# ORNL/DDStore

Hardware: AMD Instinct MI355X
Metric: samples/sec (global-shuffle sample fetch) (higher is better)
Workload: dtype bf16; 1 GPU; model=store-globalshuffle-fetch, global_batch=262144, rows_per_rank=2097152, row_bytes=512, store_dtype=f32, parallelism=dp1, mode=fetch

## Files before the change

### ddstore_amd/csrc/ddstore.hpp

```cpp
#pragma once

#include <torch/extension.h>

#include <hip/hip_runtime.h>
#include <c10/hip/HIPStream.h>
#include <ATen/Parallel.h>

#include <fcntl.h>
#include <sys/mman.h>
#include <unistd.h>

#if defined(__x86_64__)
#include <emmintrin.h>
#endif

#include <atomic>
#include <condition_variable>
#include <cstdlib>
#include <cstring>
#include <exception>
#include <functional>
#include <map>
#include <mutex>
#include <string>
// ... 417 lines not shown
                TORCH_CHECK(e == hipSuccess,
                            "ddstore open_peers: hipIpcOpenMemHandle failed for peer rank ",
                            r, " (", hipGetErrorString(e),
                            ") -- peers must share one node/xGMI domain and "
                            "HSA_ENABLE_IPC_MODE_LEGACY=0 must be set");
                v.peers[r] = p;
                v.opened[r] = 1;
            }
        }
        size_t nb = nparts_ * sizeof(void*) + (nparts_ + 1) * 8 +
                    (v.is_csr ? (nparts_ + 1) * 8 : 0) + DDS_NCTR * 8;
        HIP_CHECK(hipMalloc((void**)&v.d_peers, nb));
        v.d_prefix = reinterpret_cast<int64_t*>(v.d_peers + nparts_);
        HIP_CHECK(hipMemcpy(v.d_peers, v.peers.data(), nparts_ * sizeof(void*),
                            hipMemcpyHostToDevice));
        HIP_CHECK(hipMemcpy(v.d_prefix, v.prefix.data(), (nparts_ + 1) * 8,
                            hipMemcpyHostToDevice));
        int64_t* tail = v.d_prefix + nparts_ + 1;
        if (v.is_csr) {
            v.d_elem_prefix = tail;
            HIP_CHECK(hipMemcpy(v.d_elem_prefix, v.elem_prefix.data(),
                                (nparts_ + 1) * 8, hipMemcpyHostToDevice));
            tail += nparts_ + 1;
        }
        v.d_oob = reinterpret_cast<unsigned long long*>(tail);
        HIP_CHECK(hipMemset(v.d_oob, 0, DDS_NCTR * 8));
    }

    void update(const std::string& name, const at::Tensor& src, int64_t offset) {
        DeviceVar& v = var(name);
        TORCH_CHECK(!v.is_csr, "ddstore update: not supported for CSR variables");
        TORCH_CHECK(src.is_contiguous(), "ddstore update: array must be C-contiguous");
        TORCH_CHECK(dds_itemsize(dds_type_of(src)) == v.itemsize,
                    "ddstore update: itemsize mismatch");
        int64_t nrows = src.numel() / v.row_elems;
        TORCH_CHECK(src.numel() == nrows * v.row_elems, "ddstore update: shape mismatch");
        TORCH_CHECK(offset >= 0 && offset + nrows <= v.nrows_local,
                    "ddstore update: out of range");
        ingest(v.base, src, offset * v.row_elems * v.itemsize);
    }

    void get_range(const std::string& name, int64_t start, int64_t count,
                   at::Tensor out) {
        DeviceVar& v = var(name);
        TORCH_CHECK(!v.is_csr, "ddstore get: use get_csr for CSR variables");
        TORCH_CHECK(out.is_contiguous(), "ddstore get: output must be C-contiguous");
        TORCH_CHECK(dds_itemsize(dds_type_of(out)) == v.itemsize,
                    "ddstore get: itemsize mismatch");
        TORCH_CHECK(out.numel() == count * v.row_elems, "ddstore get: shape mismatch");
        check_peers(v);
        int64_t ntotal = v.prefix[nparts_];
        TORCH_CHECK(start >= 0 && start < ntotal, "Invalid start on target");
        int target = owner_of_host(v.prefix, start);
        TORCH_CHECK(start + count <= v.prefix[target + 1], "Invalid count on target");
        const char* src = (const char*)v.peers[target] +
                          (start - v.prefix[target]) * v.row_elems * v.itemsize;
        size_t nb = (size_t)count * v.row_elems * v.itemsize;
        if (out.device().is_cpu()) {
            HIP_CHECK(hipStreamSynchronize(stream()));
            HIP_CHECK(hipMemcpy(out.data_ptr(), src, nb, hipMemcpyDeviceToHost));
        } else {
            TORCH_CHECK(out.device().index() == device_, "ddstore get: wrong device");
            HIP_CHECK(hipMemcpyAsync(out.data_ptr(), src, nb,
                                     hipMemcpyDeviceToDevice, stream()));
        }
        v.n_gather += 1;
        v.rows_gathered += count;
        v.bytes_gathered += nb;
    }

    void gather(const std::string& name, const at::Tensor& idx, at::Tensor out) {
        RoctxRange rr_("ddstore::gather");
        DeviceVar& v = var(name);
        TORCH_CHECK(!v.is_csr, "ddstore gather: use gather_csr for CSR variables");
        check_peers(v);
        check_idx(idx);
        int64_t nidx = idx.numel();
        TORCH_CHECK(out.is_contiguous() && out.device().is_cuda() &&
                        out.device().index() == device_,
                    "ddstore gather: output must be a contiguous tensor on the store device");
        TORCH_CHECK(out.numel() == nidx * v.row_elems, "ddstore gather: shape mismatch");
        int out_t = dds_type_of(out);
        ddstore::gather_rows(stream(), (const void* const*)v.d_peers, v.d_prefix,
                             nparts_, idx.data_ptr<int64_t>(), nidx, v.row_elems,
                             v.dds_t, out_t, out.data_ptr(), v.d_oob);
        v.n_gather += 1;
        v.rows_gathered += nidx;
        v.bytes_gathered += nidx * v.row_elems * v.itemsize;
    }

    void gather_affine(const std::string& name, const at::Tensor& idx,
                       at::Tensor out, double scale, double shift) {
        RoctxRange rr_("ddstore::gather_affine");
        DeviceVar& v = var(name);
        TORCH_CHECK(!v.is_csr, "ddstore gather: use gather_csr for CSR variables");
        check_peers(v);
        check_idx(idx);
        int64_t nidx = idx.numel();
        TORCH_CHECK(out.is_contiguous() && out.device().is_cuda() &&
                        out.device().index() == device_,
                    "ddstore gather: output must be a contiguous tensor on the store device");
        TORCH_CHECK(out.numel() == nidx * v.row_elems, "ddstore gather: shape mismatch");
        int out_t = dds_type_of(out);
        TORCH_CHECK(out_t == DDS_F32 || out_t == DDS_F16 || out_t == DDS_BF16,
                    "ddstore gather: affine output must be f32/f16/bf16");
        ddstore::gather_rows_affine(stream(), (const void* const*)v.d_peers,
                                    v.d_prefix, nparts_, idx.data_ptr<int64_t>(),
                                    nidx, v.row_elems, v.dds_t, out_t,
                                    (float)scale, (float)shift, out.data_ptr(),
                                    v.d_oob);
        v.n_gather += 1;
        v.rows_gathered += nidx;
        v.bytes_gathered += nidx * v.row_elems * v.itemsize;
    }

    void gather_csr(const std::string& name, const at::Tensor& idx,
                    const at::Tensor& out_off, at::Tensor out, int64_t total_elems) {
        RoctxRange rr_("ddstore::gather_csr");
        DeviceVar& v = var(name);
        TORCH_CHECK(v.is_csr, "ddstore gather_csr: not a CSR variable");
        check_peers(v);
        check_idx(idx);
        check_idx(out_off);
        int64_t nidx = idx.numel();
        TORCH_CHECK(out_off.numel() == nidx + 1, "ddstore gather_csr: bad out_off");
        TORCH_CHECK(out.is_contiguous() && out.device().is_cuda() &&
                        dds_type_of(out) == v.dds_t,
                    "ddstore gather_csr: bad output tensor");
        TORCH_CHECK(out.numel() >= total_elems * v.row_elems,
                    "ddstore gather_csr: output too small");
        const int64_t cap = out.numel() / std::max<int64_t>(v.row_elems, 1);
        ddstore::gather_csr(stream(), (const void* const*)v.d_peers, v.d_prefix,
                            v.d_elem_prefix, nparts_, v.d_goff,
                            idx.data_ptr<int64_t>(), nidx,
                            out_off.data_ptr<int64_t>(),
                            v.row_elems * v.itemsize, cap,
                            out.data_ptr(), v.d_oob);
        v.n_gather += 1;
        v.rows_gathered += nidx;
        v.bytes_gathered += total_elems * v.row_elems * v.itemsize;
    }

    at::Tensor gather_csr_fast(const std::string& name, const at::Tensor& idx,
                               at::Tensor out) {
        RoctxRange rr_("ddstore::gather_csr_fast");
        DeviceVar& v = var(name);
        TORCH_CHECK(v.is_csr, "ddstore gather_csr: not a CSR variable");
        check_peers(v);
        check_idx(idx);
        const int64_t nidx = idx.numel();
        TORCH_CHECK(out.is_contiguous() && out.device().is_cuda() &&
                        dds_type_of(out) == v.dds_t,
                    "ddstore gather_csr: bad output tensor");
        auto opts = at::TensorOptions().dtype(at::kLong).device(idx.device());
        at::Tensor off = at::empty({nidx + 1}, opts);
        if (nidx == 0) {
            off.zero_();
            return off;
        }
        const int64_t cap = out.numel() / std::max<int64_t>(v.row_elems, 1);
        const int64_t elem_bytes = v.row_elems * v.itemsize;
        auto bopts = at::TensorOptions().dtype(at::kByte).device(idx.device());
        at::Tensor scratch = at::empty(
            {(int64_t)ddstore::csr_plan_scratch_bytes(nidx)}, bopts);
        const int64_t desc_cap =
            cap / ddstore::csr_item_elems(elem_bytes) + nidx;
        at::Tensor desc = at::empty({2 * desc_cap}, opts);
        ddstore::gather_csr_balanced(
            stream(), (const void* const*)v.d_peers, v.d_prefix,
            v.d_elem_prefix, nparts_, v.d_goff, v.prefix[nparts_],
            idx.data_ptr<int64_t>(), nidx, elem_bytes, cap,
            off.data_ptr<int64_t>(), out.data_ptr(), v.d_oob,
            scratch.data_ptr(), desc.data_ptr<int64_t>(), desc_cap);
        v.n_gather += 1;
        v.rows_gathered += nidx;
        return off;
    }

    void csr_lens(const std::string& name, const at::Tensor& idx, at::Tensor lens) {
        DeviceVar& v = var(name);
        TORCH_CHECK(v.is_csr, "ddstore csr_lens: not a CSR variable");
        check_peers(v);
        check_idx(idx);
        TORCH_CHECK(lens.scalar_type() == at::kLong && lens.is_contiguous() &&
                        lens.device().is_cuda() && lens.numel() == idx.numel(),
                    "ddstore csr_lens: bad lens tensor");
        ddstore::csr_lens(stream(), v.d_goff, idx.data_ptr<int64_t>(), idx.numel(),
                          v.prefix[nparts_], lens.data_ptr<int64_t>(), v.d_oob,
                          nullptr);
    }
// ... 686 lines not shown
```

### ddstore_amd/csrc/ddstore_kernels.h

```cpp
#pragma once

#include <hip/hip_runtime.h>
#include <cstdint>

enum DDSType : int {
    DDS_U8 = 0,
    DDS_I32 = 1,
    DDS_I64 = 2,
    DDS_F32 = 3,
    DDS_F64 = 4,
    DDS_F16 = 5,
    DDS_BF16 = 6,
    DDS_F8E4M3 = 7,
    DDS_F8E5M2 = 8,
    DDS_NUM_TYPES = 9
};

#define DDS_MAX_PARTS 128

#define DDS_CTR_OOB 0
#define DDS_CTR_CAP 1
#define DDS_CTR_ELEMS 2
#define DDS_NCTR 3

namespace ddstore {

void gather_rows(hipStream_t stream,
                 const void* const* d_peer_base,
                 const int64_t* d_prefix, int nparts,
                 const int64_t* d_idx, int64_t nidx,
                 int64_t row_elems, int in_t, int out_t,
                 void* d_out, unsigned long long* d_oob);

void gather_rows_affine(hipStream_t stream,
                        const void* const* d_peer_base,
                        const int64_t* d_prefix, int nparts,
                        const int64_t* d_idx, int64_t nidx,
                        int64_t row_elems, int in_t, int out_t,
                        float scale, float shift,
                        void* d_out, unsigned long long* d_oob);

void gather_csr(hipStream_t stream,
                const void* const* d_peer_base,
                const int64_t* d_sample_prefix,
                const int64_t* d_elem_prefix, int nparts,
                const int64_t* d_goff,
                const int64_t* d_idx, int64_t nidx,
                const int64_t* d_out_off,
                int64_t elem_bytes, int64_t cap_elems,
                void* d_out, unsigned long long* d_ctrs);

void csr_lens(hipStream_t stream, const int64_t* d_goff, const int64_t* d_idx,
              int64_t nidx, int64_t nsamples, int64_t* d_lens,
              unsigned long long* d_oob, unsigned long long* d_elems);

size_t csr_plan_scratch_bytes(int64_t nidx);
int64_t csr_item_elems(int64_t elem_bytes);
void gather_csr_balanced(hipStream_t stream, const void* const* d_peer_base,
                         const int64_t* d_sample_prefix,
                         const int64_t* d_elem_prefix, int nparts,
                         const int64_t* d_goff, int64_t nsamples_total,
                         const int64_t* d_idx, int64_t nidx,
                         int64_t elem_bytes, int64_t cap_elems,
                         int64_t* d_out_off, void* d_out,
                         unsigned long long* d_ctrs,
                         void* d_scratch, int64_t* d_desc, int64_t desc_cap);


void scatter_rows_local(hipStream_t stream,
                        void* d_base, int64_t nrows_local,
                        int64_t row_elems, int elem_t,
                        const int64_t* d_local_idx, int64_t nidx,
                        const void* d_src, unsigned long long* d_oob);

}
```

### ddstore_amd/csrc/ddstore_kernels.hip

```cpp

#include "ddstore_kernels.h"

#include <hip/hip_fp16.h>
#include <hip/hip_bf16.h>
#include <hip/hip_fp8.h>
#include <type_traits>
#include <cstdlib>

namespace ddstore {

namespace {

constexpr int kBlock = 256;
constexpr int64_t kMaxBlocks = 32768;

inline int n_blocks(int64_t work_items) {
    int64_t b = (work_items + kBlock - 1) / kBlock;
    if (b < 1) b = 1;
    if (b > kMaxBlocks) b = kMaxBlocks;
    return (int)b;
}

template <typename T, int N>
struct alignas(sizeof(T) * N) VecT {
    T v[N];
};

__device__ __forceinline__ int owner_of(const int64_t* prefix, int nparts, int64_t row) {
    int lo = 0, hi = nparts - 1;
    while (lo < hi) {
        int mid = (lo + hi + 1) >> 1;
        if (prefix[mid] <= row) lo = mid; else hi = mid - 1;
    }
    return lo;
}

template <typename T>
constexpr bool is_fp8_v =
    std::is_same_v<T, __hip_fp8_e4m3> || std::is_same_v<T, __hip_fp8_e5m2>;

template <typename Tout, typename Tin>
__device__ __forceinline__ Tout cvt(Tin v) {
    if constexpr (std::is_same_v<Tout, Tin>) {
        return v;
    } else if constexpr (std::is_same_v<Tin, __half>) {
        return cvt<Tout, float>(__half2float(v));
    } else if constexpr (std::is_same_v<Tin, __hip_bfloat16>) {
        return cvt<Tout, float>(__bfloat162float(v));
    } else if constexpr (is_fp8_v<Tin>) {
        return cvt<Tout, float>(static_cast<float>(v));
    } else if constexpr (std::is_same_v<Tout, __half>) {
        return __float2half(static_cast<float>(v));
    } else if constexpr (std::is_same_v<Tout, __hip_bfloat16>) {
        return __float2bfloat16(static_cast<float>(v));
    } else if constexpr (is_fp8_v<Tout>) {
        return Tout(static_cast<float>(v));
    } else {
        return static_cast<Tout>(v);
    }
}

template <int CHUNK>
__global__ void __launch_bounds__(kBlock)
k_gather_rows_b16(const void* const* peer_base, const int64_t* gprefix, int nparts,
                  const int64_t* idx, int64_t nidx, int64_t chunks_per_row,
                  uint4* __restrict__ out, unsigned long long* oob) {
    using V = VecT<uint4, CHUNK / 16>;
    __shared__ int64_t s_prefix[DDS_MAX_PARTS + 1];
    __shared__ const V* s_base[DDS_MAX_PARTS];
    for (int i = threadIdx.x; i <= nparts; i += kBlock) s_prefix[i] = gprefix[i];
    for (int i = threadIdx.x; i < nparts; i += kBlock)
        s_base[i] = reinterpret_cast<const V*>(peer_base[i]);
    __syncthreads();

    V* __restrict__ vout = reinterpret_cast<V*>(out);
    const int64_t total = nidx * chunks_per_row;
    for (int64_t t = (int64_t)blockIdx.x * kBlock + threadIdx.x; t < total;
         t += (int64_t)gridDim.x * kBlock) {
        const int64_t r = t / chunks_per_row;
        const int64_t c = t - r * chunks_per_row;
        const int64_t g = idx[r];
        if (g < 0 || g >= s_prefix[nparts]) {
            if (c == 0) atomicAdd(oob, 1ull);
            continue;
        }
        const int p = owner_of(s_prefix, nparts, g);
        vout[t] = s_base[p][(g - s_prefix[p]) * chunks_per_row + c];
    }
}

template <typename Tin, typename Tout>
__global__ void __launch_bounds__(kBlock)
k_gather_rows_castv(const void* const* peer_base, const int64_t* gprefix, int nparts,
                    const int64_t* idx, int64_t nidx, int64_t row_elems,
                    Tout* __restrict__ out, unsigned long long* oob) {
    constexpr int VEC = 16 / sizeof(Tout);
    using Vin = VecT<Tin, VEC>;
    using Vout = VecT<Tout, VEC>;
    __shared__ int64_t s_prefix[DDS_MAX_PARTS + 1];
    __shared__ const Tin* s_base[DDS_MAX_PARTS];
    for (int i = threadIdx.x; i <= nparts; i += kBlock) s_prefix[i] = gprefix[i];
    for (int i = threadIdx.x; i < nparts; i += kBlock)
        s_base[i] = reinterpret_cast<const Tin*>(peer_base[i]);
    __syncthreads();

    const int64_t cpr = row_elems / VEC;
    const int64_t total = nidx * cpr;
    for (int64_t t = (int64_t)blockIdx.x * kBlock + threadIdx.x; t < total;
         t += (int64_t)gridDim.x * kBlock) {
        const int64_t r = t / cpr;
        const int64_t c = t - r * cpr;
        const int64_t g = idx[r];
        if (g < 0 || g >= s_prefix[nparts]) {
            if (c == 0) atomicAdd(oob, 1ull);
            continue;
        }
        const int p = owner_of(s_prefix, nparts, g);
        const Vin vin = *reinterpret_cast<const Vin*>(
            s_base[p] + (g - s_prefix[p]) * row_elems + c * VEC);
        Vout vout;
#pragma unroll
        for (int k = 0; k < VEC; ++k) vout.v[k] = cvt<Tout>(vin.v[k]);
        *reinterpret_cast<Vout*>(out + t * VEC) = vout;
    }
}

template <typename T>
__device__ __forceinline__ float to_f32(T v) {
    if constexpr (std::is_same_v<T, __half>) return __half2float(v);
    else if constexpr (std::is_same_v<T, __hip_bfloat16>) return __bfloat162float(v);
    else if constexpr (is_fp8_v<T>) return static_cast<float>(v);
    else return (float)v;
}

template <typename Tin, typename Tout>
__global__ void __launch_bounds__(kBlock)
k_gather_rows_affine(const void* const* peer_base, const int64_t* gprefix, int nparts,
                     const int64_t* idx, int64_t nidx, int64_t row_elems,
                     float scale, float shift,
                     Tout* __restrict__ out, unsigned long long* oob) {
    constexpr int VEC = 16 / sizeof(Tout);
    using Vin = VecT<Tin, VEC>;
    using Vout = VecT<Tout, VEC>;
    __shared__ int64_t s_prefix[DDS_MAX_PARTS + 1];
    __shared__ const Tin* s_base[DDS_MAX_PARTS];
    for (int i = threadIdx.x; i <= nparts; i += kBlock) s_prefix[i] = gprefix[i];
    for (int i = threadIdx.x; i < nparts; i += kBlock)
        s_base[i] = reinterpret_cast<const Tin*>(peer_base[i]);
    __syncthreads();

    const int64_t cpr = row_elems / VEC;
    const int64_t total = nidx * cpr;
    for (int64_t t = (int64_t)blockIdx.x * kBlock + threadIdx.x; t < total;
         t += (int64_t)gridDim.x * kBlock) {
        const int64_t r = t / cpr;
        const int64_t c = t - r * cpr;
        const int64_t g = idx[r];
        if (g < 0 || g >= s_prefix[nparts]) {
            if (c == 0) atomicAdd(oob, 1ull);
            continue;
        }
        const int p = owner_of(s_prefix, nparts, g);
        const Vin vin = *reinterpret_cast<const Vin*>(
            s_base[p] + (g - s_prefix[p]) * row_elems + c * VEC);
        Vout vout;
#pragma unroll
        for (int k = 0; k < VEC; ++k)
            vout.v[k] = cvt<Tout>(fmaf(to_f32(vin.v[k]), scale, shift));
        *reinterpret_cast<Vout*>(out + t * VEC) = vout;
    }
}

template <typename Tin, typename Tout>
__global__ void __launch_bounds__(kBlock)
k_gather_rows_affine_s(const void* const* peer_base, const int64_t* gprefix, int nparts,
                       const int64_t* idx, int64_t nidx, int64_t row_elems,
                       float scale, float shift,
                       Tout* __restrict__ out, unsigned long long* oob) {
    __shared__ int64_t s_prefix[DDS_MAX_PARTS + 1];
    __shared__ const Tin* s_base[DDS_MAX_PARTS];
    for (int i = threadIdx.x; i <= nparts; i += kBlock) s_prefix[i] = gprefix[i];
    for (int i = threadIdx.x; i < nparts; i += kBlock)
        s_base[i] = reinterpret_cast<const Tin*>(peer_base[i]);
    __syncthreads();
    const int64_t total = nidx * row_elems;
    for (int64_t t = (int64_t)blockIdx.x * kBlock + threadIdx.x; t < total;
         t += (int64_t)gridDim.x * kBlock) {
        const int64_t r = t / row_elems;
        const int64_t c = t - r * row_elems;
        const int64_t g = idx[r];
        if (g < 0 || g >= s_prefix[nparts]) {
            if (c == 0) atomicAdd(oob, 1ull);
            continue;
        }
        const int p = owner_of(s_prefix, nparts, g);
        out[t] = cvt<Tout>(fmaf(
            to_f32(s_base[p][(g - s_prefix[p]) * row_elems + c]), scale, shift));
    }
}

template <typename Tin, typename Tout>
__global__ void __launch_bounds__(kBlock)
k_gather_rows_cast(const void* const* peer_base, const int64_t* gprefix, int nparts,
                   const int64_t* idx, int64_t nidx, int64_t row_elems,
                   Tout* __restrict__ out, unsigned long long* oob) {
    __shared__ int64_t s_prefix[DDS_MAX_PARTS + 1];
    __shared__ const Tin* s_base[DDS_MAX_PARTS];
    for (int i = threadIdx.x; i <= nparts; i += kBlock) s_prefix[i] = gprefix[i];
    for (int i = threadIdx.x; i < nparts; i += kBlock)
        s_base[i] = reinterpret_cast<const Tin*>(peer_base[i]);
    __syncthreads();

    const int64_t total = nidx * row_elems;
    for (int64_t t = (int64_t)blockIdx.x * kBlock + threadIdx.x; t < total;
         t += (int64_t)gridDim.x * kBlock) {
        const int64_t r = t / row_elems;
        const int64_t c = t - r * row_elems;
        const int64_t g = idx[r];
        if (g < 0 || g >= s_prefix[nparts]) {
            if (c == 0) atomicAdd(oob, 1ull);
            continue;
        }
        const int p = owner_of(s_prefix, nparts, g);
        out[t] = cvt<Tout>(s_base[p][(g - s_prefix[p]) * row_elems + c]);
    }
}

template <typename T, int GROUP>
__global__ void __launch_bounds__(kBlock)
k_gather_csr_wave(const void* const* peer_base,
                  const int64_t* sample_prefix, const int64_t* elem_prefix, int nparts,
                  const int64_t* goff,
                  const int64_t* idx, int64_t nidx,
                  const int64_t* out_off, int64_t chunks_per_elem,
                  int64_t cap_elems,
                  T* __restrict__ out, unsigned long long* ctrs) {
    __shared__ int64_t s_sprefix[DDS_MAX_PARTS + 1];
    __shared__ int64_t s_eprefix[DDS_MAX_PARTS + 1];
    __shared__ const T* s_base[DDS_MAX_PARTS];
    for (int i = threadIdx.x; i <= nparts; i += kBlock) {
        s_sprefix[i] = sample_prefix[i];
        s_eprefix[i] = elem_prefix[i];
    }
    for (int i = threadIdx.x; i < nparts; i += kBlock)
        s_base[i] = reinterpret_cast<const T*>(peer_base[i]);
    __syncthreads();

    constexpr int GPB = kBlock / GROUP;
    const int64_t first = (int64_t)blockIdx.x * GPB + threadIdx.x / GROUP;
    const int64_t step = (int64_t)gridDim.x * GPB;
    const int tid = threadIdx.x % GROUP;
    for (int64_t s = first; s < nidx; s += step) {
// ... 315 lines not shown
                   const int64_t* __restrict__ desc,
                   const int64_t* __restrict__ meta,
                   void* __restrict__ out_, unsigned long long* ctrs) {
    __shared__ const char* s_base[DDS_MAX_PARTS];
    for (int i = threadIdx.x; i < nparts; i += kBlock)
        s_base[i] = reinterpret_cast<const char*>(peer_base[i]);
    __syncthreads();
    const int64_t total = meta[0];
    constexpr int GPB = kBlock / GROUP;
    const int64_t first = (int64_t)blockIdx.x * GPB + threadIdx.x / GROUP;
    const int64_t step = (int64_t)gridDim.x * GPB;
    const int tid = threadIdx.x % GROUP;
    (void)ctrs;
    for (int64_t j = first; j < total; j += step) {
        const int64_t d0 = desc[2 * j];
        const int64_t d1 = desc[2 * j + 1];
        const int p = (int)(d0 >> 56);
        const int64_t src_u = d0 & ((int64_t(1) << 56) - 1);
        const int64_t n_u = d1 >> 44;
        const int64_t dst_u = d1 & ((int64_t(1) << 44) - 1);
        if constexpr (DW) {
            copy_dwords_store16<VAR>(
                reinterpret_cast<uint32_t*>(out_) + dst_u,
                reinterpret_cast<const uint32_t*>(s_base[p]) + src_u,
                n_u, tid, GROUP);
        } else {
            char* dst = reinterpret_cast<char*>(out_) + dst_u;
            const char* src = s_base[p] + src_u;
            for (int64_t c = tid; c < n_u; c += GROUP) dst[c] = src[c];
        }
    }
}

template <int CHUNK>
__global__ void __launch_bounds__(kBlock)
k_scatter_rows_b16(uint4* __restrict__ base_, int64_t nrows, int64_t chunks_per_row,
                   const int64_t* local_idx, int64_t nidx,
                   const uint4* __restrict__ src_, unsigned long long* oob) {
    using V = VecT<uint4, CHUNK / 16>;
    V* __restrict__ base = reinterpret_cast<V*>(base_);
    const V* __restrict__ src = reinterpret_cast<const V*>(src_);
    const int64_t total = nidx * chunks_per_row;
    for (int64_t t = (int64_t)blockIdx.x * kBlock + threadIdx.x; t < total;
         t += (int64_t)gridDim.x * kBlock) {
        const int64_t r = t / chunks_per_row;
        const int64_t c = t - r * chunks_per_row;
        const int64_t l = local_idx[r];
        if (l < 0 || l >= nrows) {
            if (c == 0) atomicAdd(oob, 1ull);
            continue;
        }
        base[l * chunks_per_row + c] = src[t];
    }
}

template <typename T>
__global__ void __launch_bounds__(kBlock)
k_scatter_rows_elem(T* __restrict__ base, int64_t nrows, int64_t row_elems,
                    const int64_t* local_idx, int64_t nidx,
                    const T* __restrict__ src, unsigned long long* oob) {
    const int64_t total = nidx * row_elems;
    for (int64_t t = (int64_t)blockIdx.x * kBlock + threadIdx.x; t < total;
         t += (int64_t)gridDim.x * kBlock) {
        const int64_t r = t / row_elems;
        const int64_t c = t - r * row_elems;
        const int64_t l = local_idx[r];
        if (l < 0 || l >= nrows) {
            if (c == 0) atomicAdd(oob, 1ull);
            continue;
        }
        base[l * row_elems + c] = src[t];
    }
}

inline int dds_itemsize(int t) {
    switch (t) {
        case DDS_U8: case DDS_F8E4M3: case DDS_F8E5M2: return 1;
        case DDS_F16: case DDS_BF16: return 2;
        case DDS_I32: case DDS_F32: return 4;
        default: return 8;
    }
}

template <typename Tin, typename Tout>
void launch_gather_cast_one(hipStream_t stream, const void* const* pb,
                            const int64_t* pf, int np, const int64_t* idx,
                            int64_t n, int64_t re, Tout* out,
                            unsigned long long* oob) {
    constexpr int VEC = 16 / sizeof(Tout);
    if (re % VEC == 0 && ((uintptr_t)out % 16) == 0) {
        const int grid = n_blocks(n * (re / VEC));
        hipLaunchKernelGGL((k_gather_rows_castv<Tin, Tout>), dim3(grid), dim3(kBlock),
                           0, stream, pb, pf, np, idx, n, re, out, oob);
    } else {
        const int grid = n_blocks(n * re);
        hipLaunchKernelGGL((k_gather_rows_cast<Tin, Tout>), dim3(grid), dim3(kBlock),
                           0, stream, pb, pf, np, idx, n, re, out, oob);
    }
}

template <typename Tin>
void launch_gather_cast_out(hipStream_t stream, const void* const* pb,
                            const int64_t* pf, int np, const int64_t* idx,
                            int64_t n, int64_t re, int out_t, void* out,
                            unsigned long long* oob) {
    switch (out_t) {
#define DDS_OUT(tag, T)                                                               \
    case tag:                                                                         \
        launch_gather_cast_one<Tin, T>(stream, pb, pf, np, idx, n, re, (T*)out, oob); \
        break;
        DDS_OUT(DDS_U8, uint8_t)
        DDS_OUT(DDS_I32, int32_t)
        DDS_OUT(DDS_I64, int64_t)
        DDS_OUT(DDS_F32, float)
        DDS_OUT(DDS_F64, double)
        DDS_OUT(DDS_F16, __half)
        DDS_OUT(DDS_BF16, __hip_bfloat16)
        DDS_OUT(DDS_F8E4M3, __hip_fp8_e4m3)
        DDS_OUT(DDS_F8E5M2, __hip_fp8_e5m2)
#undef DDS_OUT
    }
}

}

template <typename Tin>
void launch_affine_out(hipStream_t stream, const void* const* pb, const int64_t* pf,
                       int np, const int64_t* idx, int64_t n, int64_t re,
                       float a, float b, int out_t, void* out,
                       unsigned long long* oob) {
#define DDS_AFF(tag, T)                                                              \
    case tag: {                                                                      \
        constexpr int VEC = 16 / sizeof(T);                                          \
        if (re % VEC == 0 && ((uintptr_t)out % 16) == 0) {                           \
            const int grid = n_blocks(n * (re / VEC));                               \
            hipLaunchKernelGGL((k_gather_rows_affine<Tin, T>), dim3(grid),           \
                               dim3(kBlock), 0, stream, pb, pf, np, idx, n, re, a,   \
                               b, (T*)out, oob);                                     \
        } else {                                                                     \
            const int grid = n_blocks(n * re);                                       \
            hipLaunchKernelGGL((k_gather_rows_affine_s<Tin, T>), dim3(grid),         \
                               dim3(kBlock), 0, stream, pb, pf, np, idx, n, re, a,   \
                               b, (T*)out, oob);                                     \
        }                                                                            \
        break;                                                                       \
    }
    switch (out_t) {
        DDS_AFF(DDS_F32, float)
        DDS_AFF(DDS_F16, __half)
        DDS_AFF(DDS_BF16, __hip_bfloat16)
    }
#undef DDS_AFF
}

void gather_rows_affine(hipStream_t stream,
                        const void* const* d_peer_base,
                        const int64_t* d_prefix, int nparts,
                        const int64_t* d_idx, int64_t nidx,
                        int64_t row_elems, int in_t, int out_t,
                        float scale, float shift,
                        void* d_out, unsigned long long* d_oob) {
    if (nidx == 0 || row_elems == 0) return;
    switch (in_t) {
#define DDS_AIN(tag, T)                                                          \
    case tag:                                                                    \
        launch_affine_out<T>(stream, d_peer_base, d_prefix, nparts, d_idx,       \
                             nidx, row_elems, scale, shift, out_t, d_out,        \
                             d_oob);                                             \
        break;
        DDS_AIN(DDS_U8, uint8_t)
        DDS_AIN(DDS_I32, int32_t)
        DDS_AIN(DDS_I64, int64_t)
        DDS_AIN(DDS_F32, float)
        DDS_AIN(DDS_F64, double)
        DDS_AIN(DDS_F16, __half)
        DDS_AIN(DDS_BF16, __hip_bfloat16)
        DDS_AIN(DDS_F8E4M3, __hip_fp8_e4m3)
        DDS_AIN(DDS_F8E5M2, __hip_fp8_e5m2)
#undef DDS_AIN
    }
}

void gather_rows(hipStream_t stream,
                 const void* const* d_peer_base,
                 const int64_t* d_prefix, int nparts,
                 const int64_t* d_idx, int64_t nidx,
                 int64_t row_elems, int in_t, int out_t,
                 void* d_out, unsigned long long* d_oob) {
    if (nidx == 0 || row_elems == 0) return;
    const int64_t row_bytes = row_elems * dds_itemsize(in_t);
    const uintptr_t out_align = (uintptr_t)d_out;
    if (in_t == out_t && row_bytes % 16 == 0 && out_align % 16 == 0) {
        const int64_t cpr = row_bytes / 16;
        if (row_bytes % 32 == 0 && row_bytes >= 128 && out_align % 32 == 0) {
            const int64_t cpr32 = row_bytes / 32;
            const int grid = n_blocks(nidx * cpr32);
            hipLaunchKernelGGL((k_gather_rows_b16<32>), dim3(grid), dim3(kBlock), 0,
                               stream, d_peer_base, d_prefix, nparts, d_idx, nidx,
                               cpr32, (uint4*)d_out, d_oob);
        } else {
            const int grid = n_blocks(nidx * cpr);
            hipLaunchKernelGGL((k_gather_rows_b16<16>), dim3(grid), dim3(kBlock), 0,
                               stream, d_peer_base, d_prefix, nparts, d_idx, nidx,
                               cpr, (uint4*)d_out, d_oob);
        }
        return;
    }
    switch (in_t) {
#define DDS_IN(tag, T)                                                           \
    case tag:                                                                    \
        launch_gather_cast_out<T>(stream, d_peer_base, d_prefix, nparts, d_idx,  \
                                  nidx, row_elems, out_t, d_out, d_oob);         \
        break;
        DDS_IN(DDS_U8, uint8_t)
        DDS_IN(DDS_I32, int32_t)
        DDS_IN(DDS_I64, int64_t)
        DDS_IN(DDS_F32, float)
        DDS_IN(DDS_F64, double)
        DDS_IN(DDS_F16, __half)
        DDS_IN(DDS_BF16, __hip_bfloat16)
        DDS_IN(DDS_F8E4M3, __hip_fp8_e4m3)
        DDS_IN(DDS_F8E5M2, __hip_fp8_e5m2)
#undef DDS_IN
    }
}

void csr_lens(hipStream_t stream, const int64_t* d_goff, const int64_t* d_idx,
              int64_t nidx, int64_t nsamples, int64_t* d_lens,
              unsigned long long* d_oob, unsigned long long* d_elems) {
    if (nidx == 0) return;
    hipLaunchKernelGGL(k_csr_lens, dim3(n_blocks(nidx)), dim3(kBlock), 0, stream,
                       d_goff, d_idx, nidx, nsamples, d_lens, d_oob, d_elems);
}


void gather_csr(hipStream_t stream,
                const void* const* d_peer_base,
                const int64_t* d_sample_prefix,
                const int64_t* d_elem_prefix, int nparts,
                const int64_t* d_goff,
                const int64_t* d_idx, int64_t nidx,
                const int64_t* d_out_off,
                int64_t elem_bytes, int64_t cap_elems,
                void* d_out, unsigned long long* d_ctrs) {
    if (nidx == 0) return;
    static const int g_override = [] {
        const char* e = getenv("DDSTORE_CSR_GROUP");
        return e ? atoi(e) : 0;
    }();
    int group = nidx >= 16384 ? 16 : (nidx >= 4096 ? 64 : 256);
    if (g_override) group = g_override;
    int64_t b = (nidx + (kBlock / group) - 1) / (kBlock / group);
    const int grid = (int)(b < kMaxBlocks ? b : kMaxBlocks);
    const uintptr_t oa = (uintptr_t)d_out;
#define DDS_CSR_G(T, div, G)                                                         \
    hipLaunchKernelGGL((k_gather_csr_wave<T, G>), dim3(grid), dim3(kBlock), 0,       \
                       stream, d_peer_base, d_sample_prefix, d_elem_prefix, nparts,  \
                       d_goff, d_idx, nidx, d_out_off, elem_bytes / div, cap_elems,  \
                       (T*)d_out, d_ctrs)
#define DDS_CSR_T(T, div)                                                            \
    do {                                                                             \
        if (group == 8) DDS_CSR_G(T, div, 8);                                        \
        else if (group == 16) DDS_CSR_G(T, div, 16);                                  \
        else if (group == 32) DDS_CSR_G(T, div, 32);                                 \
        else if (group == 64) DDS_CSR_G(T, div, 64);                                 \
        else DDS_CSR_G(T, div, 256);                                                 \
    } while (0)
    static const int copy_var = [] {
        const char* e = getenv("DDSTORE_CSR_COPY");
        int v = e ? atoi(e) : 0;
        return (v >= 0 && v <= 2) ? v : 0;
    }();
#define DDS_CSR_DW_V(G, V)                                                           \
    hipLaunchKernelGGL((k_gather_csr_dw<G, V>), dim3(grid), dim3(kBlock), 0, stream, \
                       d_peer_base, d_sample_prefix, d_elem_prefix, nparts, d_goff,  \
                       d_idx, nidx, d_out_off, elem_bytes / 4, cap_elems,            \
                       (uint32_t*)d_out, d_ctrs)
#define DDS_CSR_DW(G)                                                                \
    do {                                                                             \
        if (copy_var == 0) DDS_CSR_DW_V(G, 0);                                       \
        else if (copy_var == 2) DDS_CSR_DW_V(G, 2);                                  \
        else DDS_CSR_DW_V(G, 1);                                                     \
    } while (0)
    if (elem_bytes % 16 == 0 && oa % 16 == 0) {
        DDS_CSR_T(uint4, 16);
    } else if (elem_bytes % 4 == 0 && oa % 4 == 0) {
        if (group == 8) DDS_CSR_DW(8);
        else if (group == 16) DDS_CSR_DW(16);
        else if (group == 32) DDS_CSR_DW(32);
        else if (group == 64) DDS_CSR_DW(64);
        else DDS_CSR_DW(256);
    } else {
        DDS_CSR_T(uint8_t, 1);
    }
// ... 117 lines not shown
```

Before: 6.240 billion samples/s.

## Add wave-tiled gather kernel with kernel-arg directory and nontemporal stores

Adds a new gather kernel in which each wavefront handles a tile of rows. It loads the row indices once per lane, prefetches the next tile's indices, resolves each row's owner partition from a directory passed as kernel arguments (for up to 8 parts) instead of a shared-memory binary search, and broadcasts source pointers with shuffles. Loads are unrolled and outputs use nontemporal 16-byte stores. The identity, cast and affine gather paths all route to this kernel by default, with environment knobs to fall back. The aim is to cut per-element index loads, directory lookups and the cost of the integer division in the old grid-stride kernel. In exchange the grid is limited to 8 blocks per CU, which may reduce memory parallelism.

```diff
diff --git a/ddstore_amd/csrc/ddstore.hpp b/ddstore_amd/csrc/ddstore.hpp
--- a/ddstore_amd/csrc/ddstore.hpp
+++ b/ddstore_amd/csrc/ddstore.hpp
@@ -523,6 +523,7 @@
         TORCH_CHECK(out.numel() == nidx * v.row_elems, "ddstore gather: shape mismatch");
         int out_t = dds_type_of(out);
         ddstore::gather_rows(stream(), (const void* const*)v.d_peers, v.d_prefix,
+                             (const void* const*)v.peers.data(), v.prefix.data(),
                              nparts_, idx.data_ptr<int64_t>(), nidx, v.row_elems,
                              v.dds_t, out_t, out.data_ptr(), v.d_oob);
         v.n_gather += 1;
@@ -546,7 +547,8 @@
         TORCH_CHECK(out_t == DDS_F32 || out_t == DDS_F16 || out_t == DDS_BF16,
                     "ddstore gather: affine output must be f32/f16/bf16");
         ddstore::gather_rows_affine(stream(), (const void* const*)v.d_peers,
-                                    v.d_prefix, nparts_, idx.data_ptr<int64_t>(),
+                                    v.d_prefix, (const void* const*)v.peers.data(),
+                                    v.prefix.data(), nparts_, idx.data_ptr<int64_t>(),
                                     nidx, v.row_elems, v.dds_t, out_t,
                                     (float)scale, (float)shift, out.data_ptr(),
                                     v.d_oob);
diff --git a/ddstore_amd/csrc/ddstore_kernels.h b/ddstore_amd/csrc/ddstore_kernels.h
--- a/ddstore_amd/csrc/ddstore_kernels.h
+++ b/ddstore_amd/csrc/ddstore_kernels.h
@@ -23,18 +23,29 @@
 #define DDS_CTR_ELEMS 2
 #define DDS_NCTR 3
 
+#define DDS_DIR_KPARTS 8
+
 namespace ddstore {
+
+struct GatherDirK {
+    int64_t prefix[DDS_DIR_KPARTS + 1];
+    const void* base[DDS_DIR_KPARTS];
+};
 
 void gather_rows(hipStream_t stream,
                  const void* const* d_peer_base,
-                 const int64_t* d_prefix, int nparts,
+                 const int64_t* d_prefix,
+                 const void* const* h_peer_base,
+                 const int64_t* h_prefix, int nparts,
                  const int64_t* d_idx, int64_t nidx,
                  int64_t row_elems, int in_t, int out_t,
                  void* d_out, unsigned long long* d_oob);
 
 void gather_rows_affine(hipStream_t stream,
                         const void* const* d_peer_base,
-                        const int64_t* d_prefix, int nparts,
+                        const int64_t* d_prefix,
+                        const void* const* h_peer_base,
+                        const int64_t* h_prefix, int nparts,
                         const int64_t* d_idx, int64_t nidx,
                         int64_t row_elems, int in_t, int out_t,
                         float scale, float shift,
diff --git a/ddstore_amd/csrc/ddstore_kernels.hip b/ddstore_amd/csrc/ddstore_kernels.hip
--- a/ddstore_amd/csrc/ddstore_kernels.hip
+++ b/ddstore_amd/csrc/ddstore_kernels.hip
@@ -6,6 +6,7 @@
 #include <hip/hip_fp8.h>
 #include <type_traits>
 #include <cstdlib>
+#include <string>
 
 namespace ddstore {
 
@@ -168,6 +169,182 @@
         for (int k = 0; k < VEC; ++k)
             vout.v[k] = cvt<Tout>(fmaf(to_f32(vin.v[k]), scale, shift));
         *reinterpret_cast<Vout*>(out + t * VEC) = vout;
+    }
+}
+
+struct XfIdentity {
+    template <typename Tout, typename Tin>
+    __device__ __forceinline__ Tout apply(Tin v) const { return v; }
+};
+struct XfCast {
+    template <typename Tout, typename Tin>
+    __device__ __forceinline__ Tout apply(Tin v) const { return cvt<Tout>(v); }
+};
+struct XfAffine {
+    float scale, shift;
+    template <typename Tout, typename Tin>
+    __device__ __forceinline__ Tout apply(Tin v) const {
+        return cvt<Tout>(fmaf(to_f32(v), scale, shift));
+    }
+};
+
+typedef uint32_t dds_u32x4 __attribute__((ext_vector_type(4)));
+typedef uint32_t dds_u32x2 __attribute__((ext_vector_type(2)));
+#define DDS_GLOBAL_AS __attribute__((address_space(1)))
+
+template <typename V>
+__device__ __forceinline__ void store_out(V* p, const V& v) {
+    static_assert(sizeof(V) == 16, "store side is exactly 16 B per lane");
+    dds_u32x4 w;
+    __builtin_memcpy(&w, &v, 16);
+    __builtin_nontemporal_store(w, reinterpret_cast<dds_u32x4*>(p));
+}
+
+template <typename V>
+__device__ __forceinline__ V load_global(uintptr_t a) {
+    constexpr int B = sizeof(V);
+    V r;
+    if constexpr (B % 16 == 0) {
+        dds_u32x4 w[B / 16];
+#pragma unroll
+        for (int i = 0; i < B / 16; ++i)
+            w[i] = ((const DDS_GLOBAL_AS dds_u32x4*)a)[i];
+        __builtin_memcpy(&r, w, B);
+    } else if constexpr (B == 8) {
+        const dds_u32x2 w = *(const DDS_GLOBAL_AS dds_u32x2*)a;
+        __builtin_memcpy(&r, &w, B);
+    } else if constexpr (B == 4) {
+        const uint32_t w = *(const DDS_GLOBAL_AS uint32_t*)a;
+        __builtin_memcpy(&r, &w, B);
+    } else {
+        static_assert(B == 2, "unsupported vector size");
+        const uint16_t w = *(const DDS_GLOBAL_AS uint16_t*)a;
+        __builtin_memcpy(&r, &w, B);
+    }
+    return r;
+}
+
+template <int INB>
+constexpr int tiled_unroll() {
+    return INB >= 128 ? 1 : (128 / INB > 8 ? 8 : 128 / INB);
+}
+
+template <typename Tin, typename Tout, typename Xf, bool LDSDIR>
+__global__ void __launch_bounds__(kBlock)
+k_gather_tiled(const GatherDirK dir, const void* const* peer_base,
+               const int64_t* gprefix, int nparts,
+               const int64_t* __restrict__ idx, int64_t nidx, int64_t ntiles,
+               uint32_t cpr, uint32_t tile_rows, Xf xf,
+               Tout* __restrict__ out, unsigned long long* oob) {
+    constexpr int VEC = 16 / sizeof(Tout);
+    constexpr int INB = VEC * sizeof(Tin);
+    constexpr int U = tiled_unroll<INB>();
+    using Vin = VecT<Tin, VEC>;
+    using Vout = VecT<Tout, VEC>;
+    __shared__ int64_t s_prefix[LDSDIR ? DDS_MAX_PARTS + 1 : 1];
+    __shared__ uintptr_t s_base[LDSDIR ? DDS_MAX_PARTS : 1];
+    if constexpr (LDSDIR) {
+        for (int i = threadIdx.x; i <= nparts; i += kBlock) s_prefix[i] = gprefix[i];
+        for (int i = threadIdx.x; i < nparts; i += kBlock)
+            s_base[i] = reinterpret_cast<uintptr_t>(peer_base[i]);
+        __syncthreads();
+    }
+    const int64_t total = LDSDIR ? s_prefix[nparts] : dir.prefix[DDS_DIR_KPARTS];
+
+    const uint32_t lane = threadIdx.x & 63;
+    const uint32_t wave = __builtin_amdgcn_readfirstlane(threadIdx.x >> 6);
+    const int64_t wstride = (int64_t)gridDim.x * (kBlock / 64);
+    int64_t tile = (int64_t)blockIdx.x * (kBlock / 64) + wave;
+    if (tile >= ntiles) return;
+
+    const uint32_t q64 = 64u / cpr, r64 = 64u % cpr;
+    const uint32_t rl0 = lane / cpr, c0 = lane - rl0 * cpr;
+    const int64_t row_bytes = (int64_t)cpr * INB;
+
+    int64_t g_next = 0;
+    {
+        const int64_t r = tile * tile_rows + lane;
+        if (lane < tile_rows && r < nidx) g_next = idx[r];
+    }
+    for (; tile < ntiles; tile += wstride) {
+        const int64_t row0 = tile * tile_rows;
+        const int64_t left = nidx - row0;
+        const uint32_t nrows = left < (int64_t)tile_rows ? (uint32_t)left : tile_rows;
+        const int64_t g = g_next;
+        if (tile + wstride < ntiles) {
+            const int64_t r = (tile + wstride) * tile_rows + lane;
+            if (lane < tile_rows && r < nidx) g_next = idx[r];
+        }
+        uintptr_t src = 0;
+        if (lane < nrows) {
+            if (g < 0 || g >= total) {
+                atomicAdd(oob, 1ull);
+            } else if constexpr (LDSDIR) {
+                const int p = owner_of(s_prefix, nparts, g);
+                src = s_base[p] + (uintptr_t)((g - s_prefix[p]) * row_bytes);
+            } else {
+                int64_t pf = dir.prefix[0];
+                uintptr_t bs = reinterpret_cast<uintptr_t>(dir.base[0]);
+#pragma unroll
+                for (int k = 1; k < DDS_DIR_KPARTS; ++k) {
+                    const bool ge = dir.prefix[k] <= g;
+                    pf = ge ? dir.prefix[k] : pf;
+                    bs = ge ? reinterpret_cast<uintptr_t>(dir.base[k]) : bs;
+                }
+                src = bs + (uintptr_t)((g - pf) * row_bytes);
+            }
+        }
+        Vout* __restrict__ op = reinterpret_cast<Vout*>(out) + row0 * cpr;
+        const uint32_t nch = nrows * cpr;
+        const bool clean = __ballot(lane < nrows && src == 0) == 0;
+        uint32_t rl = rl0, c = c0;
+        for (uint32_t jb = 0; jb < nch; jb += 64u * U) {
+            if (clean && jb + 64u * U <= nch) {
+                Vin vin[U];
+#pragma unroll
+                for (int u = 0; u < U; ++u) {
+                    const uintptr_t sp =
+                        (uintptr_t)__shfl((unsigned long long)src, (int)(rl & 63u));
+                    vin[u] = load_global<Vin>(sp + (uintptr_t)(c * (uint32_t)INB));
+                    c += r64;
+                    rl += q64;
+                    if (c >= cpr) {
+                        c -= cpr;
+                        rl += 1;
+                    }
+                }
+#pragma unroll
+                for (int u = 0; u < U; ++u) {
+                    Vout vout;
+#pragma unroll
+                    for (int k = 0; k < VEC; ++k)
+                        vout.v[k] = xf.template apply<Tout>(vin[u].v[k]);
+                    store_out(&op[jb + 64u * u + lane], vout);
+                }
+            } else {
+#pragma unroll 1
+                for (int u = 0; u < U; ++u) {
+                    const uint32_t j = jb + 64u * u + lane;
+                    const uintptr_t sp =
+                        (uintptr_t)__shfl((unsigned long long)src, (int)(rl & 63u));
+                    if (j < nch && sp != 0) {
+                        const Vin v =
+                            load_global<Vin>(sp + (uintptr_t)(c * (uint32_t)INB));
+                        Vout vout;
+#pragma unroll
+                        for (int k = 0; k < VEC; ++k)
+                            vout.v[k] = xf.template apply<Tout>(v.v[k]);
+                        store_out(&op[j], vout);
+                    }
+                    c += r64;
+                    rl += q64;
+                    if (c >= cpr) {
+                        c -= cpr;
+                        rl += 1;
+                    }
+                }
+            }
+        }
     }
 }
 
@@ -649,12 +826,111 @@
     }
 }
 
+struct DirArgs {
+    const void* const* d_pb;
+    const int64_t* d_pf;
+    const void* const* h_pb;
+    const int64_t* h_pf;
+    int np;
+};
+
+struct GatherKnobs {
+    int kernel = 0;
+    int blocks = 0;
+    bool dir_lds = false;
+    int tile_rows = 64;
+};
+const GatherKnobs& gather_knobs() {
+    static const GatherKnobs k = [] {
+        GatherKnobs g;
+        if (const char* e = getenv("DDSTORE_GATHER_KERNEL")) {
+            const std::string s(e);
+            g.kernel = s == "legacy" ? 1 : (s == "tiled" ? 2 : 0);
+        }
+        if (const char* e = getenv("DDSTORE_GATHER_BLOCKS")) {
+            const int v = atoi(e);
+            if (v > 0) g.blocks = v;
+        }
+        if (const char* e = getenv("DDSTORE_GATHER_DIR"))
+            g.dir_lds = std::string(e) == "lds";
+        if (const char* e = getenv("DDSTORE_GATHER_TILE_ROWS")) {
+            const int v = atoi(e);
+            if (v >= 1 && v <= 64) g.tile_rows = v;
+        }
+        return g;
+    }();
+    return k;
+}
+
+int cu_count() {
+    static const int n = [] {
+        int dev = 0, v = 0;
+        if (hipGetDevice(&dev) != hipSuccess ||
+            hipDeviceGetAttribute(&v, hipDeviceAttributeMultiprocessorCount, dev) !=
+                hipSuccess || v <= 0)
+            v = 256;
+        return v;
+    }();
+    return n;
+}
+
+constexpr int kBlocksPerCU = 8;
+constexpr int kTilesPerWave = 2;
+constexpr int64_t kTiledMaxCpr = 4096;
+constexpr int64_t kTiledMinCpr = 8;
+
+template <typename Tin, typename Tout, typename Xf>
+bool launch_tiled(hipStream_t stream, const DirArgs& d, const int64_t* idx,
+                  int64_t n, int64_t re, Xf xf, Tout* out,
+                  unsigned long long* oob) {
+    constexpr int VEC = 16 / sizeof(Tout);
+    constexpr int INB = VEC * (int)sizeof(Tin);
+    constexpr int U = tiled_unroll<INB>();
+    const GatherKnobs& kn = gather_knobs();
+    if (kn.kernel == 1 || re % VEC != 0 || ((uintptr_t)out % 16) != 0) return false;
+    const int64_t cpr = re / VEC;
+    if (cpr > kTiledMaxCpr) return false;
+    if (kn.kernel != 2 && cpr < kTiledMinCpr) return false;
+
+    int64_t blocks_max = (int64_t)cu_count() * kBlocksPerCU;
+    if (kn.blocks > 0) blocks_max = kn.blocks;
+    int64_t tr_min = (64 * U + cpr - 1) / cpr;
+    int64_t tr = n / (blocks_max * (kBlock / 64) * kTilesPerWave);
+    if (tr < tr_min) tr = tr_min;
+    if (tr > kn.tile_rows) tr = kn.tile_rows;
+    const int64_t ntiles = (n + tr - 1) / tr;
+    int64_t grid = (ntiles + (kBlock / 64) - 1) / (kBlock / 64);
+    if (grid > blocks_max) grid = blocks_max;
+
+    if (d.np <= DDS_DIR_KPARTS && !kn.dir_lds) {
+        GatherDirK dir;
+        const int64_t total = d.h_pf[d.np];
+        for (int k = 0; k <= DDS_DIR_KPARTS; ++k)
+            dir.prefix[k] = k < d.np ? d.h_pf[k] : total;
+        for (int k = 0; k < DDS_DIR_KPARTS; ++k)
+            dir.base[k] = k < d.np ? d.h_pb[k] : nullptr;
+        hipLaunchKernelGGL((k_gather_tiled<Tin, Tout, Xf, false>), dim3((unsigned)grid),
+                           dim3(kBlock), 0, stream, dir, d.d_pb, d.d_pf, d.np, idx, n,
+                           ntiles, (uint32_t)cpr, (uint32_t)tr, xf, out, oob);
+    } else {
+        GatherDirK dir = {};
+        hipLaunchKernelGGL((k_gather_tiled<Tin, Tout, Xf, true>), dim3((unsigned)grid),
+                           dim3(kBlock), 0, stream, dir, d.d_pb, d.d_pf, d.np, idx, n,
+                           ntiles, (uint32_t)cpr, (uint32_t)tr, xf, out, oob);
+    }
+    return true;
+}
+
 template <typename Tin, typename Tout>
-void launch_gather_cast_one(hipStream_t stream, const void* const* pb,
-                            const int64_t* pf, int np, const int64_t* idx,
+void launch_gather_cast_one(hipStream_t stream, const DirArgs& d,
+                            const int64_t* idx,
                             int64_t n, int64_t re, Tout* out,
                             unsigned long long* oob) {
     constexpr int VEC = 16 / sizeof(Tout);
+    if (launch_tiled<Tin, Tout>(stream, d, idx, n, re, XfCast{}, out, oob)) return;
+    const void* const* pb = d.d_pb;
+    const int64_t* pf = d.d_pf;
+    const int np = d.np;
     if (re % VEC == 0 && ((uintptr_t)out % 16) == 0) {
         const int grid = n_blocks(n * (re / VEC));
         hipLaunchKernelGGL((k_gather_rows_castv<Tin, Tout>), dim3(grid), dim3(kBlock),
@@ -667,14 +943,14 @@
 }
 
 template <typename Tin>
-void launch_gather_cast_out(hipStream_t stream, const void* const* pb,
-                            const int64_t* pf, int np, const int64_t* idx,
+void launch_gather_cast_out(hipStream_t stream, const DirArgs& d,
+                            const int64_t* idx,
                             int64_t n, int64_t re, int out_t, void* out,
                             unsigned long long* oob) {
     switch (out_t) {
 #define DDS_OUT(tag, T)                                                               \
     case tag:                                                                         \
-        launch_gather_cast_one<Tin, T>(stream, pb, pf, np, idx, n, re, (T*)out, oob); \
+        launch_gather_cast_one<Tin, T>(stream, d, idx, n, re, (T*)out, oob);          \
         break;
         DDS_OUT(DDS_U8, uint8_t)
         DDS_OUT(DDS_I32, int32_t)
@@ -692,14 +968,19 @@
 }
 
 template <typename Tin>
-void launch_affine_out(hipStream_t stream, const void* const* pb, const int64_t* pf,
-                       int np, const int64_t* idx, int64_t n, int64_t re,
+void launch_affine_out(hipStream_t stream, const DirArgs& d,
+                       const int64_t* idx, int64_t n, int64_t re,
                        float a, float b, int out_t, void* out,
                        unsigned long long* oob) {
+    const void* const* pb = d.d_pb;
+    const int64_t* pf = d.d_pf;
+    const int np = d.np;
 #define DDS_AFF(tag, T)                                                              \
     case tag: {                                                                      \
         constexpr int VEC = 16 / sizeof(T);                                          \
-        if (re % VEC == 0 && ((uintptr_t)out % 16) == 0) {                           \
+        if (launch_tiled<Tin, T>(stream, d, idx, n, re, XfAffine{a, b}, (T*)out,     \
+                                 oob)) {                                             \
+        } else if (re % VEC == 0 && ((uintptr_t)out % 16) == 0) {                    \
             const int grid = n_blocks(n * (re / VEC));                               \
             hipLaunchKernelGGL((k_gather_rows_affine<Tin, T>), dim3(grid),           \
                                dim3(kBlock), 0, stream, pb, pf, np, idx, n, re, a,   \
@@ -722,16 +1003,19 @@
 
 void gather_rows_affine(hipStream_t stream,
                         const void* const* d_peer_base,
-                        const int64_t* d_prefix, int nparts,
+                        const int64_t* d_prefix,
+                        const void* const* h_peer_base,
+                        const int64_t* h_prefix, int nparts,
                         const int64_t* d_idx, int64_t nidx,
                         int64_t row_elems, int in_t, int out_t,
                         float scale, float shift,
                         void* d_out, unsigned long long* d_oob) {
     if (nidx == 0 || row_elems == 0) return;
+    const DirArgs dir{d_peer_base, d_prefix, h_peer_base, h_prefix, nparts};
     switch (in_t) {
 #define DDS_AIN(tag, T)                                                          \
     case tag:                                                                    \
-        launch_affine_out<T>(stream, d_peer_base, d_prefix, nparts, d_idx,       \
+        launch_affine_out<T>(stream, dir, d_idx,                                 \
                              nidx, row_elems, scale, shift, out_t, d_out,        \
                              d_oob);                                             \
         break;
@@ -750,15 +1034,21 @@
 
 void gather_rows(hipStream_t stream,
                  const void* const* d_peer_base,
-                 const int64_t* d_prefix, int nparts,
+                 const int64_t* d_prefix,
+                 const void* const* h_peer_base,
+                 const int64_t* h_prefix, int nparts,
                  const int64_t* d_idx, int64_t nidx,
                  int64_t row_elems, int in_t, int out_t,
                  void* d_out, unsigned long long* d_oob) {
     if (nidx == 0 || row_elems == 0) return;
+    const DirArgs dir{d_peer_base, d_prefix, h_peer_base, h_prefix, nparts};
     const int64_t row_bytes = row_elems * dds_itemsize(in_t);
     const uintptr_t out_align = (uintptr_t)d_out;
     if (in_t == out_t && row_bytes % 16 == 0 && out_align % 16 == 0) {
         const int64_t cpr = row_bytes / 16;
+        if (launch_tiled<uint32_t, uint32_t>(stream, dir, d_idx, nidx, row_bytes / 4,
+                                             XfIdentity{}, (uint32_t*)d_out, d_oob))
+            return;
         if (row_bytes % 32 == 0 && row_bytes >= 128 && out_align % 32 == 0) {
             const int64_t cpr32 = row_bytes / 32;
             const int grid = n_blocks(nidx * cpr32);
@@ -776,7 +1066,7 @@
     switch (in_t) {
 #define DDS_IN(tag, T)                                                           \
     case tag:                                                                    \
-        launch_gather_cast_out<T>(stream, d_peer_base, d_prefix, nparts, d_idx,  \
+        launch_gather_cast_out<T>(stream, dir, d_idx,                            \
                                   nidx, row_elems, out_t, d_out, d_oob);         \
         break;
         DDS_IN(DDS_U8, uint8_t)
```

Measured after the change: 6.808 billion samples/s (median of 6 runs). 1.09x the previous value.
